# luciddreamer-cvlab/LucidDreamer

Hardware: AMD Instinct MI355X
Metric: views/sec fwd+bwd @1080p (1e6 Gaussians) (higher is better)
Workload: dtype f32

## Files before the change

### luciddreamer_amd/build.py

```python
import os
import shutil
import subprocess
import sys

_HERE = os.path.dirname(os.path.abspath(__file__))
CSRC = os.path.join(_HERE, "csrc")
LIBDIR = os.path.join(_HERE, "lib")
OBJDIR = os.path.join(LIBDIR, "obj")
LIB_PATH = os.path.join(LIBDIR, "liblucid_raster.so")
INCLUDE = os.path.join(os.path.dirname(_HERE), "include")

COMMON_FLAGS = ["--offload-arch=gfx950", "-O3", "-std=c++17", "-fPIC", "-munsafe-fp-atomics",
                "-fno-gpu-rdc", "-Wall", "-Wno-unused-function", "-I", INCLUDE]
SOURCES = {
    "preprocess.hip": ["-ffp-contract=off", "-fno-slp-vectorize"],
    "binning.hip": [],
    "tilebin.hip": [],
    "render_fwd.hip": ["-fno-slp-vectorize"],
    "render_bwd.hip": ["-fno-slp-vectorize"],
    "gauss_bwd.hip": [],
    "knn.hip": [],
    "loss.hip": ["-fno-slp-vectorize"],
    "rows.hip": [],
    "adam.hip": [],
    "mcmc.hip": [],
    "filter3d.hip": ["-ffp-contract=off"],
    "video.hip": ["-ffp-contract=off"],
    "api.hip": [],
}


def hipcc():
    for cand in (os.environ.get("HIPCC"), shutil.which("hipcc"), "/opt/rocm/bin/hipcc"):
        if cand and os.path.exists(cand):
            return cand
    raise RuntimeError("hipcc not found (need ROCm >= 7.0 with gfx950 support)")


def _stale(target, deps):
    if not os.path.exists(target):
        return True
    t = os.path.getmtime(target)
    return any(os.path.getmtime(d) > t for d in deps)


def source_hash():
    import hashlib
    h = hashlib.sha1()
    names = sorted(f for f in os.listdir(CSRC) if f.endswith((".hip", ".h", ".cpp")))
    for path in [os.path.join(CSRC, f) for f in names] + [os.path.join(INCLUDE, "lucid_raster.h")]:
        h.update(os.path.basename(path).encode())
        with open(path, "rb") as f:
            h.update(f.read())
    return h.hexdigest()[:12]


def _write_hash_header():
    path = os.path.join(OBJDIR, "lr_src_hash.h")
    text = f'#define LR_SRC_HASH "{source_hash()}"\n'
    old = open(path).read() if os.path.exists(path) else None
    if old != text:
        with open(path, "w") as f:
            f.write(text)
    return path


DIAG_LIBDIR = os.path.join(_HERE, "lib_diag")


def build(force=False, verbose=False, diagnostics=False):
    libdir = DIAG_LIBDIR if diagnostics else LIBDIR
    objdir = os.path.join(libdir, "obj")
    lib_path = os.path.join(libdir, "liblucid_raster.so")
    os.makedirs(objdir, exist_ok=True)
    os.makedirs(OBJDIR, exist_ok=True)
    cc = hipcc()
    hash_header = _write_hash_header()
    headers = [os.path.join(CSRC, "common.h"), os.path.join(CSRC, "gauss_bwd_body.h"), os.path.join(CSRC, "loss_ssim_fwd_body.h"),
               os.path.join(CSRC, "loss_ssim_bwd_body.h"), os.path.join(INCLUDE, "lucid_raster.h"), os.path.abspath(__file__)]
    objs = []
    procs = []
    for src, extra in SOURCES.items():
        sp = os.path.join(CSRC, src)
        op = os.path.join(objdir, src.replace(".hip", ".o"))
        if diagnostics:
            extra = extra + ["-DLR_DIAGNOSTICS"]
        objs.append(op)
        deps = [sp] + headers + ([hash_header] if src == "api.hip" else [])
        if force or _stale(op, deps):
            cmd = [cc, "-c", sp, "-o", op] + COMMON_FLAGS + ["-I", OBJDIR] + extra + os.environ.get("LR_EXTRA_HIPCC_FLAGS", "").split()
            if verbose:
                print(" ".join(cmd), flush=True)
            procs.append((src, subprocess.Popen(cmd, stdout=subprocess.PIPE, stderr=subprocess.STDOUT, text=True)))
    failed = []
    for src, p in procs:
        out, _ = p.communicate()
        if p.returncode != 0:
            failed.append((src, out))
        elif verbose and out.strip():
            print(out)
    if failed:
        raise RuntimeError("hipcc failed:\n" + "\n".join(f"--- {s} ---\n{o}" for s, o in failed))
    if force or procs or _stale(lib_path, objs):
        cmd = [cc, "-shared", "-fPIC", "--offload-arch=gfx950", "-o", lib_path] + objs
        if verbose:
            print(" ".join(cmd), flush=True)
        subprocess.check_call(cmd)
    return lib_path


EXT_SRC = os.path.join(CSRC, "torch_ext.cpp")


def ext_path():
    import sysconfig
    return os.path.join(_HERE, "_C_ext" + sysconfig.get_config_var("EXT_SUFFIX"))


def build_ext(force=False, verbose=False):
    import sysconfig
    import torch
    from torch.utils import cpp_extension as ce
    out = ext_path()
    deps = [EXT_SRC, os.path.join(INCLUDE, "lucid_raster.h"), os.path.abspath(__file__)]
    if not force and not _stale(out, deps):
        return out
    rocm = os.environ.get("ROCM_PATH", "/opt/rocm")
    cmd = ["g++", "-O2", "-std=c++17", "-fPIC", "-shared", "-w", EXT_SRC, "-o", out,
           "-DTORCH_EXTENSION_NAME=_C_ext", "-DTORCH_API_INCLUDE_EXTENSION_H", "-DUSE_ROCM", "-D__HIP_PLATFORM_AMD__",
           f"-D_GLIBCXX_USE_CXX11_ABI={int(torch._C._GLIBCXX_USE_CXX11_ABI)}", "-I", INCLUDE, "-I", os.path.join(rocm, "include"),
           "-I", sysconfig.get_paths()["include"]]
# ... 19 lines not shown
```

### luciddreamer_amd/csrc/api.hip

```cpp
#include "common.h"
#include "../../include/lucid_raster.h"
#include "lr_src_hash.h"

#include <cstdio>
#include <cstdlib>
#include <cstddef>
#include <cstring>
#include <cmath>
#include <map>
#include <atomic>
#include <chrono>
#include <mutex>
#include <thread>
#include <string>
#include <vector>

namespace {

thread_local std::string g_last_error;

int fail(int code, const std::string& msg)
{
    g_last_error = msg;
    return code;
// ... 15 lines not shown
            if (e__ == hipSuccess) e__ = hipGetLastError();                                       \
            if (e__ != hipSuccess)                                                                \
                return fail(LR_ERR_HIP, std::string("[HIP ERROR] after ") + what + ": " + hipGetErrorString(e__)); \
        }                                                                                         \
    } while (0)

enum Stage { ST_PREPROCESS = 0, ST_COMPACT, ST_BIN_COUNT, ST_BIN_SCAN, ST_BIN_SCATTER, ST_TILE_SORT, ST_RENDER_FWD,
             ST_GRAD_ZERO, ST_RENDER_BWD, ST_OUT_ZERO, ST_GAUSS_BWD, ST_COUNT };
const char* const kStageNames[ST_COUNT] = { "preprocess", "compact", "bin_count", "bin_scan", "bin_scatter", "tile_sort",
                                            "render_fwd", "grad_zero", "render_bwd", "out_zero", "gauss_bwd" };
struct ProfRec { int stage; hipEvent_t e0, e1; };
bool g_prof_on = false;
std::mutex g_prof_mu;
std::vector<ProfRec> g_prof_recs;
std::vector<hipEvent_t> g_prof_pool;

hipEvent_t prof_event()
{
    {
        std::lock_guard<std::mutex> lock(g_prof_mu);
        if (!g_prof_pool.empty()) { hipEvent_t e = g_prof_pool.back(); g_prof_pool.pop_back(); return e; }
    }
    hipEvent_t e = nullptr;
    (void)hipEventCreate(&e);
    return e;
}
struct ProfScope {
    hipStream_t s; ProfRec r; bool on;
    ProfScope(int stage, hipStream_t s_) : s(s_), on(g_prof_on)
    {
        if (on) { r.stage = stage; r.e0 = prof_event(); r.e1 = prof_event(); (void)hipEventRecord(r.e0, s); }
    }
    ~ProfScope()
    {
        if (on) { (void)hipEventRecord(r.e1, s); std::lock_guard<std::mutex> lock(g_prof_mu); g_prof_recs.push_back(r); }
    }
};

struct BinProf : lr::TileBinTimes {
    ProfRec cur; bool open = false;
    void mark(int boundary, hipStream_t s) override
    {
        if (!g_prof_on) return;
        if (open) { (void)hipEventRecord(cur.e1, s); std::lock_guard<std::mutex> lock(g_prof_mu); g_prof_recs.push_back(cur); open = false; }
        if (boundary < 4) {
            cur.stage = ST_BIN_COUNT + boundary; cur.e0 = prof_event(); cur.e1 = prof_event();
            (void)hipEventRecord(cur.e0, s); open = true;
        }
    }
};

struct TuneTable { int v[lr::TUNE_COUNT]; TuneTable() { for (int& x : v) x = -1; } } g_tune_table;
int* const g_tune = g_tune_table.v;
const char* const kTuneNames[] = { "bwd_red", "blend_quad", "tile_map", "preprocess", "gauss_bwd", "tsort", "walk_own", "hit_mask", "views_in_flight", "strict", "part_scan", "bwd_seg", "fwd_pair" };
static_assert(sizeof(kTuneNames) / sizeof(kTuneNames[0]) == lr::TUNE_COUNT, "one name per TuneKey");

std::mutex g_hint_mu;
std::map<std::pair<int, uint32_t>, float> g_vis_frac;
std::map<std::pair<int, uint32_t>, uint32_t> g_inst_hint;
constexpr float kSparseViewFraction = 0.30f;

void view_hint_note(int device, uint32_t P, uint32_t num_compact, uint32_t num_instances)
{
    if (P == 0) return;
    std::lock_guard<std::mutex> lock(g_hint_mu);
    g_vis_frac[std::make_pair(device, P)] = (float)num_compact / (float)P;
    g_inst_hint[std::make_pair(device, P)] = num_instances;
}
long long view_hint_instances(int device, uint32_t P)
{
    std::lock_guard<std::mutex> lock(g_hint_mu);
    auto it = g_inst_hint.find(std::make_pair(device, P));
    return it != g_inst_hint.end() ? (long long)it->second : -1;
}
bool view_hint_sparse(int device, uint32_t P)
{
    std::lock_guard<std::mutex> lock(g_hint_mu);
    auto it = g_vis_frac.find(std::make_pair(device, P));
    return it != g_vis_frac.end() && it->second <= kSparseViewFraction;
}

thread_local bool g_early_request = false;
thread_local long long g_early_ticket = -1;

struct StreamScratch { uint32_t* words = nullptr; size_t n = 0; bool dirty = false; };
std::mutex g_scratch_mu;
std::map<std::pair<int, hipStream_t>, StreamScratch> g_scratch;
StreamScratch* stream_scratch(hipStream_t s, size_t n_words)
{
    int device = 0;
    if (hipGetDevice(&device) != hipSuccess) return nullptr;
    StreamScratch* sc;
    {
        std::lock_guard<std::mutex> lock(g_scratch_mu);
        sc = &g_scratch[std::make_pair(device, s)];
    }
    if (sc->n < n_words) {
        uint32_t* w = nullptr;
        const size_t cap = n_words + n_words / 2 + 64;
        if (hipMalloc(reinterpret_cast<void**>(&w), cap * 4) != hipSuccess) return nullptr;
        if (hipMemsetAsync(w, 0, cap * 4, s) != hipSuccess) return nullptr;
        sc->words = w; sc->n = cap; sc->dirty = false;
    } else if (sc->dirty) {
        if (hipMemsetAsync(sc->words, 0, sc->n * 4, s) != hipSuccess) return nullptr;
        sc->dirty = false;
    }
    return sc;
// ... 130 lines not shown
    if (v.raw && M < 1) return fail(LR_ERR_INVALID_ARG, "raw mode: M = 1 + number of features_rest coefficients must be >= 1");
    if (P < 0 || width <= 0 || height <= 0) return fail(LR_ERR_INVALID_ARG, "P, width, height must be positive");
    if (!a.geom_alloc || !a.binning_alloc || !a.img_alloc) return fail(LR_ERR_INVALID_ARG, "allocator callbacks are required");
    if (!v.background || !v.viewmatrix || !v.projmatrix || !v.campos || !a.out_color || (!a.out_depth && !depth_optional))
        return fail(LR_ERR_INVALID_ARG, "background/viewmatrix/projmatrix/cam_pos/out_color/out_depth are required");
    if (P > 0 && (!v.means3D || !v.opacities || !radii)) return fail(LR_ERR_INVALID_ARG, "means3D/opacities/radii are required");
    if (P > 0 && v.shs == nullptr && v.colors_precomp == nullptr)
        return fail(LR_ERR_INVALID_ARG, "For non-RGB, provide precomputed Gaussian colors!");
    if (P > 0 && v.cov3D_precomp == nullptr && (v.scales == nullptr || v.rotations == nullptr))
        return fail(LR_ERR_INVALID_ARG, "provide scales+rotations or cov3D_precomp");
    if (v.shs != nullptr && (D < 0 || D > 3 || (D + 1) * (D + 1) > M))
        return fail(LR_ERR_INVALID_ARG, "SH degree must be 0..3 and (D+1)^2 <= M");
    if (binning_capacity < 0 || binning_capacity > 0xFFFFFFF0ll) return fail(LR_ERR_INVALID_ARG, "bad binning_capacity");

    const int gx = (width + TILE_X - 1) / TILE_X, gy = (height + TILE_Y - 1) / TILE_Y;
    const int num_tiles = gx * gy;

    const GeomLayout GL = geom_layout(P);
    const ImgLayout IL = img_layout(width, height);
    char* geom = a.geom_alloc(GL.total, a.geom_user);
    char* img = a.img_alloc(IL.total, a.img_user);
    if (!geom || !img) return fail(LR_ERR_ALLOC, "geom/img allocator returned NULL");

    GeomHeader* hdr = reinterpret_cast<GeomHeader*>(geom + GL.header);
    GaussRec* rec = reinterpret_cast<GaussRec*>(geom + GL.rec);
    uint8_t* clamped = reinterpret_cast<uint8_t*>(geom + GL.clamped);
    uint32_t* tiles_touched = reinterpret_cast<uint32_t*>(geom + GL.tiles_touched);
    uint32_t* vis_list = reinterpret_cast<uint32_t*>(geom + GL.vis_list);
    uint32_t* offsets = reinterpret_cast<uint32_t*>(geom + GL.offsets);
    uint4* hitrec = reinterpret_cast<uint4*>(geom + GL.hitrec);
    float* final_T = reinterpret_cast<float*>(img + IL.final_T);
    uint32_t* n_contrib = reinterpret_cast<uint32_t*>(img + IL.n_contrib);
    uint2* ranges = reinterpret_cast<uint2*>(img + IL.ranges);
    uint32_t* part_hist = reinterpret_cast<uint32_t*>(img + IL.part_hist);
    uint32_t* bin_total = reinterpret_cast<uint32_t*>(img + IL.bin_total);
    uint32_t* bin_start = reinterpret_cast<uint32_t*>(img + IL.bin_start);
    uint32_t* big_queue = reinterpret_cast<uint32_t*>(img + IL.big_queue);

    const size_t n_sum_words = chunk_sum_words(P);
    StreamScratch* scratch = P > 0 ? stream_scratch(s, n_sum_words) : nullptr;
    if (P > 0 && !scratch) return fail(LR_ERR_ALLOC, "could not allocate the per-stream scratch");
    struct DirtyOnError { StreamScratch* sc; bool armed; ~DirtyOnError() { if (sc && armed) sc->dirty = true; } } guard{ scratch, false };
    g_last_forward_ticket = -1;

    ViewParams vp;
    vp.view = v.viewmatrix; vp.proj = v.projmatrix; vp.campos = v.campos;
    vp.tan_fovx = v.tan_fovx; vp.tan_fovy = v.tan_fovy;
    vp.focal_y = height / (2.0f * v.tan_fovy);
    vp.focal_x = width / (2.0f * v.tan_fovx);
    vp.scale_modifier = v.scale_modifier;
    vp.W = width; vp.H = height; vp.gx = gx; vp.gy = gy; vp.P = P; vp.D = D; vp.M = M;
    vp.hit_origin_limit = tune_get(TUNE_HIT_MASK) == 0 ? 0 : HIT_ORIGIN_LIMIT;
    vp.raw = v.raw != 0; vp.sh_rest = v.sh_rest; vp.opacity_raw = nullptr; vp.dL_dsh_rest = nullptr;

    long long R_bound = 0;
    int num_rendered = 0;
    uint32_t* point_list = nullptr;
    uint32_t* inst_gid = nullptr;
    uint32_t* list_gid = nullptr;
    uint8_t* quad_hits = nullptr;
    uint2* seg_list = nullptr;
    float4* ckpt = nullptr;
    bool ranges_written = false;
    long long inst_hint = -1;

    if (P > 0) {
        int device = 0;
        (void)hipGetDevice(&device);
        inst_hint = view_hint_instances(device, (uint32_t)P);
        { ProfScope ps(ST_PREPROCESS, s);
        launch_preprocess(vp, v.means3D, v.scales, v.rotations, v.opacities, v.shs, v.cov3D_precomp, v.colors_precomp,
                          a.prefiltered != 0, radii, rec, clamped, tiles_touched, hitrec, nullptr, hdr,
                          (uint32_t)binning_capacity, scratch->words,
                          view_hint_sparse(device, (uint32_t)P), s, antialiasing); }
        guard.armed = true;
        LR_DEBUG_SYNC(debug, s, "preprocess");

        uint32_t* log_slot = nullptr;
        uint32_t log_tag = 0;
#ifdef LR_DIAGNOSTICS
        static const bool no_log = [] { const char* e = getenv("LR_NO_FWD_LOG"); return e && atoi(e) != 0; }();
#else
        constexpr bool no_log = false;
#endif
        if (binning_capacity != 0 && !no_log) {
            if (ForwardLog* L = forward_log(device)) {
                const long long seq = L->next.fetch_add(1);
                log_slot = L->dev + (size_t)(seq % kLogSlots) * kLogWords;
                log_tag = (uint32_t)(seq + 1);
                g_last_forward_ticket = ((long long)device << 41) | kLogTicketBit | (seq & (kLogTicketBit - 1));
            }
        }
        { ProfScope ps(ST_COMPACT, s);
        launch_compact(P, tiles_touched, reinterpret_cast<const uint4*>(scratch->words), vis_list, offsets, hdr,
                       (uint32_t)binning_capacity, log_slot, log_tag, bin_total, (uint32_t)part_plan(num_tiles).bins, reset_sticky, s); }
        LR_DEBUG_SYNC(debug, s, "compact");

        if (binning_capacity == 0) {
            uint32_t meta[9];
            LR_HIP_CHECK(hipMemcpyAsync(meta, hdr, sizeof(meta), hipMemcpyDeviceToHost, s));
            LR_HIP_CHECK(hipStreamSynchronize(s));
            view_hint_note(device, (uint32_t)P, meta[8], meta[6]);
            R_bound = meta[6];
            if (meta[0] > 0x7FFFFFFFu)
                return fail(LR_ERR_INVALID_ARG, "num_rendered exceeds INT_MAX: use async mode (binning_capacity > 0) and read the count with lr_check");
            num_rendered = (int)meta[0];
// ... 58 lines not shown
    using namespace lr;
    const bool antialiasing = g_antialiasing.load(std::memory_order_relaxed) != 0;
    const lr_view& v = a.view;
    const int P = v.P, M = v.M, width = v.width, height = v.height, debug = a.debug;
    const bool raw = v.raw != 0;
    char* const geom_buffer = a.geom_buffer; char* const binning_buffer = a.binning_buffer; char* const image_buffer = a.image_buffer;
    const unsigned int accumulate_mask = a.accumulate_mask;
    const bool depth = a.dL_depths != nullptr && a.depth_image != nullptr;
    hipStream_t s = reinterpret_cast<hipStream_t>(a.stream);
    if (P <= 0) return 0;
    if (!geom_buffer || !binning_buffer || !image_buffer) return fail(LR_ERR_INVALID_ARG, "scratch buffers are required");
    if (!a.dL_dpix || !a.dL_dmean2D || !a.dL_dopacity || !a.dL_dmean3D)
        return fail(LR_ERR_INVALID_ARG, "gradient outputs dL_dmean2D/dL_dopacity/dL_dmean3D are required");
    if (v.colors_precomp != nullptr && !a.dL_dcolor) return fail(LR_ERR_INVALID_ARG, "dL_dcolor is required with colors_precomp");
    if (v.cov3D_precomp != nullptr && !a.dL_dcov3D) return fail(LR_ERR_INVALID_ARG, "dL_dcov3D is required with cov3D_precomp");
    if (v.scales != nullptr && (!a.dL_dscale || !a.dL_drot)) return fail(LR_ERR_INVALID_ARG, "dL_dscale/dL_drot are required with scales");
    if (v.shs != nullptr && a.dL_dsh == nullptr) return fail(LR_ERR_INVALID_ARG, "dL_dsh is required when shs is given");
    {
        const void* g16[11] = { a.dL_dmean2D, a.dL_dconic, a.dL_dopacity, a.dL_dcolor, a.dL_dmean3D, a.dL_dcov3D, a.dL_dsh, a.dL_dscale,
                                a.dL_drot, a.dL_dsh_rest, a.dL_dmean2D_abs };
        for (const void* p : g16)
            if ((reinterpret_cast<uintptr_t>(p) & 15u) != 0)
                return fail(LR_ERR_INVALID_ARG, "gradient outputs must be 16-byte aligned");
    }

    const int gx = (width + TILE_X - 1) / TILE_X, gy = (height + TILE_Y - 1) / TILE_Y;
    const GeomLayout GL = geom_layout(P);
    const ImgLayout IL = img_layout(width, height);
    const GaussRec* rec = reinterpret_cast<const GaussRec*>(geom_buffer + GL.rec);
    const uint8_t* clamped = reinterpret_cast<const uint8_t*>(geom_buffer + GL.clamped);
    const uint32_t* offsets = reinterpret_cast<const uint32_t*>(geom_buffer + GL.offsets);
    const uint32_t* vis_list = reinterpret_cast<const uint32_t*>(geom_buffer + GL.vis_list);
    const GeomHeader* hdr = reinterpret_cast<const GeomHeader*>(geom_buffer + GL.header);
    const float* final_T = reinterpret_cast<const float*>(image_buffer + IL.final_T);
    const uint32_t* n_contrib = reinterpret_cast<const uint32_t*>(image_buffer + IL.n_contrib);
    const uint2* ranges = reinterpret_cast<const uint2*>(image_buffer + IL.ranges);

    const uint32_t* point_list = reinterpret_cast<const uint32_t*>(binning_buffer);
    const long long seg_bound = (a.binning_capacity > 0 || a.R > 0)
                                    ? bin_seg_capacity(a.binning_capacity > 0 ? a.binning_capacity : (long long)a.R) : -1;

    ViewParams vp;
    vp.view = v.viewmatrix; vp.proj = v.projmatrix; vp.campos = v.campos;
    vp.tan_fovx = v.tan_fovx; vp.tan_fovy = v.tan_fovy;
    vp.focal_y = height / (2.0f * v.tan_fovy);
    vp.focal_x = width / (2.0f * v.tan_fovx);
    vp.scale_modifier = v.scale_modifier;
    vp.W = width; vp.H = height; vp.gx = gx; vp.gy = gy; vp.P = P; vp.D = v.D; vp.M = M;
    vp.hit_origin_limit = tune_get(TUNE_HIT_MASK) == 0 ? 0 : HIT_ORIGIN_LIMIT;
    vp.raw = raw;
    vp.sh_rest = raw ? v.sh_rest : nullptr;
    vp.opacity_raw = raw ? v.opacities : nullptr;
    vp.dL_dsh_rest = raw ? a.dL_dsh_rest : nullptr;

    { ProfScope ps(ST_RENDER_BWD, s);
    launch_render_bwd(width, height, gx, gy, ranges, point_list, rec, v.background, final_T, n_contrib, a.dL_dpix,
                      binning_buffer, hdr, reinterpret_cast<const uint32_t*>(image_buffer + IL.tile_seg0),
                      reinterpret_cast<const float4*>(image_buffer + IL.c_final), seg_bound, s,
                      depth ? a.dL_depths : nullptr, depth ? a.depth_image : nullptr, a.dL_dalpha, a.dL_dmean2D_abs != nullptr || stat_abs); }
    LR_DEBUG_SYNC(debug, s, "render backward");
    if (debug) {
        uint32_t uncovered = 0;
        LR_HIP_CHECK(hipMemcpy(&uncovered, &hdr->bwd_uncovered, 4, hipMemcpyDeviceToHost));
        if (uncovered) return fail(LR_ERR_INVALID_ARG, kUncoveredMsg);
    }
    if (wait_before_accumulate != nullptr) LR_HIP_CHECK(hipStreamWaitEvent(s, wait_before_accumulate, 0));
    {
        const unsigned long long Pn = (unsigned long long)P;
        float* ptrs[9] = { a.dL_dmean2D, a.dL_dconic, a.dL_dopacity, a.dL_dcolor, a.dL_dmean3D, a.dL_dcov3D, a.dL_dsh, a.dL_dscale, a.dL_drot };
        const unsigned long long nsh = raw ? 3 * Pn : (unsigned long long)M * 3 * Pn;
        const unsigned long long nf[9] = { 3 * Pn, 4 * Pn, Pn, 3 * Pn, 3 * Pn, 6 * Pn, nsh, 3 * Pn, 4 * Pn };
        float* zp[11]; unsigned long long zn[11]; int zc = 0;
        const bool no_fill = (accumulate_mask & LR_ACC_NO_ZERO_FILL) != 0u;
        for (int k = 0; k < 9; k++)
            if (ptrs[k] != nullptr && !((accumulate_mask >> k) & 1u) && (!no_fill || k == ACC_MEAN2D)) { zp[zc] = ptrs[k]; zn[zc] = nf[k]; zc++; }
        if (!no_fill && raw && a.dL_dsh_rest != nullptr && M > 1 && !((accumulate_mask >> ACC_SH) & 1u) && zc < 9) {
            zp[zc] = a.dL_dsh_rest; zn[zc] = (unsigned long long)(M - 1) * 3 * Pn; zc++;
        }
        const bool abs_own = a.dL_dmean2D_abs != nullptr && zc >= 9;
        if (a.dL_dmean2D_abs != nullptr && !abs_own) { zp[zc] = a.dL_dmean2D_abs; zn[zc] = 3 * Pn; zc++; }
        if (zc > 0) {
            ProfScope ps(ST_OUT_ZERO, s);
            launch_zero_outputs(zp, zn, zc, s);
            if (abs_own) { float* one = a.dL_dmean2D_abs; const unsigned long long n = 3 * Pn; launch_zero_outputs(&one, &n, 1, s); }
        }
    }
    { ProfScope ps(ST_GAUSS_BWD, s);
    launch_gauss_bwd(vp, v.means3D, v.scales, v.rotations, v.shs, v.cov3D_precomp, v.colors_precomp, vis_list, clamped, offsets,
                     binning_buffer, hdr,
                     a.dL_dmean2D, a.dL_dconic, a.dL_dopacity, a.dL_dcolor, a.dL_dmean3D, a.dL_dcov3D, a.dL_dsh, a.dL_dscale,
                     a.dL_drot, accumulate_mask, acc16, s, depth, antialiasing, a.dL_dmean2D_abs, stat_accum, stat_abs); }
    LR_DEBUG_SYNC(debug, s, "preprocess backward");
    LR_HIP_CHECK(hipGetLastError());
    return 0;
}

static int check_backward(const lr_backward_args& a)
{
    const lr_view& v = a.view;
    if (const int rc = check_view(v)) return rc;
    if (!v.raw && a.dL_dsh_rest) return fail(LR_ERR_INVALID_ARG, "dL_dsh_rest goes with raw mode only");
    if (v.P > 0 && a.dL_depths != nullptr && a.depth_image == nullptr)
        return fail(LR_ERR_INVALID_ARG, "lr_view_backward: dL_depths needs the forward's depth image");
    if (v.raw && v.P > 0 && (!a.dL_dsh || (v.M > 1 && !a.dL_dsh_rest)))
        return fail(LR_ERR_INVALID_ARG, "raw mode needs dL_dfeatures_dc and dL_dfeatures_rest");
    return 0;
// ... 995 lines not shown
```

### luciddreamer_amd/csrc/common.h

```cpp
#pragma once
#include <hip/hip_runtime.h>
#include <stdint.h>
#include <stddef.h>

namespace lr {

constexpr int TILE_X = 16;
constexpr int TILE_Y = 16;
constexpr int TILE_PIX = TILE_X * TILE_Y;
constexpr int WAVE = 64;

struct __attribute__((aligned(16))) GaussRec {
    float x, y, ca, cb;
    float cc, opacity, r, g;
    float b, depth, qmax, pad1;
};
static_assert(sizeof(GaussRec) == 48, "GaussRec must be 48 bytes");

struct __attribute__((aligned(16))) GradRec {
    float dmx, dmy, dca, dcb;
    float dcc, dop, dr, dg;
    float db, pad0, pad1, pad2;
};
static_assert(sizeof(GradRec) == 48, "GradRec must be 48 bytes");

constexpr uint32_t HIT_MASK_TILES = 64;
constexpr int HIT_ORIGIN_LIMIT = 4096;
__host__ __device__ inline uint32_t hit_geo(int minx, int miny, int rw, uint32_t area, int origin_limit)
{
    return (area <= HIT_MASK_TILES && minx < origin_limit && miny < origin_limit)
               ? ((uint32_t)minx | ((uint32_t)miny << 12) | ((uint32_t)rw << 24)) : 0u;
}

struct GeomHeader {
    uint32_t num_rendered;
    uint32_t overflow;
    uint32_t prefilter_trap;
    uint32_t capacity;
    uint32_t P;
    uint32_t num_sorted;
    uint32_t num_instances;
    uint32_t bin_bound;
    uint32_t num_compact;
    uint32_t n_seg;
    uint32_t bwd_uncovered;
    uint32_t reserved[49];
    uint32_t sticky_overflow;
    uint32_t reserved_tail[3];
};
static_assert(sizeof(GeomHeader) == 256, "GeomHeader must be 256 bytes");

__device__ __forceinline__ void lds_barrier()
{
    asm volatile("s_waitcnt lgkmcnt(0)" ::: "memory");
    __syncthreads();
}
// ... 153 lines not shown
    return t * dy;
}
__device__ __forceinline__ float gauss_power1(float Ap, float Bd, float Cdd, float dx)
{
    return __builtin_fmaf(__builtin_fmaf(Ap, dx, Bd), dx, Cdd);
}
template <bool STRICT>
__device__ __forceinline__ void gauss_row(float qB, float qC, float dy, float& r0, float& r1)
{
    if (STRICT) { r0 = dy; r1 = 0.f; }
    else { r0 = gauss_bd(qB, dy); r1 = gauss_cdd(qC, dy); }
}
__device__ __forceinline__ float gauss_power_strict(float ca, float cb, float cc, float dx, float dy)
{
#pragma clang fp contract(off)
    return -0.5f * (ca * dx * dx + cc * dy * dy) - cb * dx * dy;
}
__device__ __forceinline__ float strict_expf(float x)
{
#pragma clang fp contract(off)
    const float c = 0x1.715476p+0f, cc = 0x1.4ae0bep-26f;
    const float ph = x * c;
    const float pl = __builtin_fmaf(x, cc, __builtin_fmaf(x, c, -ph));
    const float e = __builtin_rintf(ph);
    const float a = (ph - e) + pl;
    return __builtin_ldexpf(__builtin_amdgcn_exp2f(a), (int)e);
}
template <bool STRICT>
__device__ __forceinline__ float gauss_weight(float qA, float qB, float qC, float r0, float r1, float dx, float& power)
{
    if (STRICT) {
        power = gauss_power_strict(qA, qB, qC, dx, r0);
        return strict_expf(power);
    }
    power = gauss_power1(qA, r0, r1, dx);
    return __builtin_amdgcn_exp2f(power);
}

constexpr float LOG2E = 1.4426950408889634f;
constexpr float LN2 = 0.6931471805599453f;
__device__ __forceinline__ float gauss_exp2(float power2) { return __builtin_amdgcn_exp2f(power2); }

struct ViewParams {
    const float* view;
    const float* proj;
    const float* campos;
    float tan_fovx, tan_fovy, focal_x, focal_y, scale_modifier;
    int W, H, gx, gy, P, D, M;
    int hit_origin_limit;
    int raw;
    const float* sh_rest;
    const float* opacity_raw;
    float* dL_dsh_rest;
};

__device__ __forceinline__ float act_scale(float s) { return expf(s); }
__device__ __forceinline__ float act_opacity(float o) { return 1.0f / (1.0f + expf(-o)); }
__device__ __forceinline__ float act_quat_inv_norm(float r, float x, float y, float z)
{
    return 1.0f / fmaxf(sqrtf(r * r + x * x + y * y + z * z), 1e-12f);
}

void launch_preprocess(const ViewParams& vp, const float* means3D, const float* scales, const float* rotations,
                       const float* opacities, const float* shs, const float* cov3D_precomp,
                       const float* colors_precomp, bool prefiltered, int* radii, GaussRec* rec,
                       uint8_t* clamped, uint32_t* tiles_touched, uint4* hitrec, uint32_t* depth_key,
                       GeomHeader* hdr, uint32_t binning_capacity, uint32_t* chunk_sums, bool sparse_view_hint, hipStream_t s,
                       bool antialiasing = false);
inline size_t chunk_sum_words(int P) { return 4 * (((size_t)(P > 0 ? P : 1) + SCAN_TILE - 1) / SCAN_TILE) + 1; }
void launch_mark_visible(int P, const float* means3D, const float* view, const float* proj, uint8_t* present,
                         hipStream_t s);

inline int radix_sort_passes(int end_bit) { return (end_bit + RADIX_BITS - 1) / RADIX_BITS; }
void radix_sort_pairs(uint32_t* key_a, uint32_t* key_b, uint32_t* val_a, uint32_t* val_b, bool vals_iota,
                      const uint32_t* n_dev, long long n_bound, int end_bit, uint32_t* hist,
                      uint32_t** keys_out, uint32_t** vals_out, hipStream_t s);

void launch_compact(int P, const uint32_t* tiles_touched, const uint4* block_sums,
                    uint32_t* vis_list, uint32_t* offsets, GeomHeader* hdr, uint32_t capacity, uint32_t* log_slot,
                    uint32_t log_tag, uint32_t* zero_words, uint32_t n_zero, bool reset_sticky, hipStream_t s);
struct TileBinTimes { virtual void mark(int boundary, hipStream_t s) = 0; virtual ~TileBinTimes() {} };
int launch_tile_binning(int P, int gx, int gy, int slot_bits, const uint32_t* vis_list, const uint32_t* offsets,
                        const uint4* hitrec, const GaussRec* rec, const int* radii, GeomHeader* hdr,
                        uint32_t* part_hist, uint32_t* bin_total, uint32_t* bin_start, uint32_t* big_queue,
                        uint32_t* inst_gid, unsigned long long* words, uint32_t* point_list, uint32_t* list_gid, uint2* ranges,
                        long long bin_bound_hint, TileBinTimes* t, uint32_t* clear_words, uint32_t n_clear, hipStream_t s);

enum TuneKey { TUNE_BWD_RED = 0, TUNE_BLEND_QUAD, TUNE_TILE_MAP, TUNE_PREPROCESS, TUNE_GAUSS_BWD, TUNE_TSORT, TUNE_WALK_OWN, TUNE_HIT_MASK, TUNE_VIEWS_IN_FLIGHT, TUNE_STRICT, TUNE_PART_SCAN, TUNE_BWD_SEG, TUNE_FWD_PAIR, TUNE_COUNT };
int tune_get(int key);

enum { BLEND_HALF = 0, BLEND_QUAD = 1, BLEND_TILE = 2 };
int blend_shape(int num_tiles, long long inst_bound = -1);
struct ViewsInFlight { explicit ViewsInFlight(int n); ~ViewsInFlight(); int prev; };
int views_in_flight();
void note_fwd_shape(int shape);
int last_fwd_shape();
int last_bwd_shape();
enum { TILE_MAP_BANDS = 0, TILE_MAP_PLAIN = 1 };
int blend_tile_map(int num_tiles);
__device__ __forceinline__ int blend_tile(int map, int num_tiles)
{
    int t = (int)blockIdx.x;
    if (map == TILE_MAP_BANDS) {
        const int per = (num_tiles + 7) >> 3;
        t = (int)(blockIdx.x & 7) * per + (int)(blockIdx.x >> 3);
    }
    return t < num_tiles ? t : -1;
}
void launch_render_fwd(int W, int H, int gx, int gy, const uint2* ranges, const uint32_t* point_list,
                       const uint32_t* list_gid, const GaussRec* rec, const float* bg, float* final_T,
                       uint32_t* n_contrib, float* out_color, float* out_depth, uint8_t* quad_hits,
                       GeomHeader* hdr, uint2* seg_list, float4* ckpt, uint32_t* tile_seg0, float4* c_final,
                       long long inst_hint, hipStream_t s);
void launch_render_alpha(const float* final_T, long long n, float* alpha, hipStream_t s);
void launch_render_bwd(int W, int H, int gx, int gy, const uint2* ranges, const uint32_t* point_list,
                       const GaussRec* rec, const float* bg, const float* final_T,
                       const uint32_t* n_contrib, const float* dL_dpix, char* bin_base, const GeomHeader* hdr,
                       const uint32_t* tile_seg0, const float4* c_final, long long seg_bound, hipStream_t s,
                       const float* dL_ddepth = nullptr, const float* depth_img = nullptr, const float* dL_dalpha = nullptr,
                       bool absgrad = false);
__device__ __forceinline__ void adam_one(float gi, float& mi, float& vi, float& pi, float w1, float beta2, float w2,
                                         float bc2_sqrt, float eps, float step_size)
{
    mi = __builtin_fmaf(w1, gi - mi, mi);
    vi = vi * beta2;
    vi = __builtin_fmaf(w2 * gi, gi, vi);
    const float denom = sqrtf(vi) / bc2_sqrt + eps;
    pi = __builtin_fmaf(-step_size, mi / denom, pi);
}
void launch_gauss_bwd(const ViewParams& vp, const float* means3D, const float* scales, const float* rotations,
                      const float* shs, const float* cov3D_precomp, const float* colors_precomp,
                      const uint32_t* vis_list, const uint8_t* clamped, const uint32_t* offsets,
                      const char* bin_base, const GeomHeader* hdr,
                      float* dL_dmean2D, float* dL_dconic, float* dL_dopacity, float* dL_dcolor,
                      float* dL_dmean3D, float* dL_dcov3D, float* dL_dsh, float* dL_dscale, float* dL_drot,
                      uint32_t accum_mask, float* acc16, hipStream_t s, bool depth = false, bool antialiasing = false,
                      float* dL_dmean2D_abs = nullptr, float* stat_accum = nullptr, bool stat_abs = false);
void launch_uninterleave_add(int P, const float* acc16, float* mean2D, float* opacity, float* mean3D, float* scale, float* rot,
                             hipStream_t s, float* stat_accum = nullptr);
size_t select_workspace_bytes(int P);
int launch_select_rows(int P, const uint8_t* mask, int n_tensors, const void* const* src, void* const* dst,
// ... 82 lines not shown
```

### luciddreamer_amd/csrc/preprocess.hip

```cpp
#include <cstddef>
#include "common.h"

namespace lr {

namespace {

__device__ constexpr float SH_C0 = 0.28209479177387814f;
__device__ constexpr float SH_C1 = 0.4886025119029199f;
__device__ constexpr float SH_C2[5] = { 1.0925484305920792f, -1.0925484305920792f, 0.31539156525252005f,
                                        -1.0925484305920792f, 0.5462742152960396f };
__device__ constexpr float SH_C3[7] = { -0.5900435899266435f, 2.890611442640554f, -0.4570457994644658f,
                                        0.3731763325901154f, -0.4570457994644658f, 1.445305721320277f,
                                        -0.5900435899266435f };

struct M3 { float c[3][3]; };

__device__ __forceinline__ M3 m3_mul(const M3& A, const M3& B)
{
    M3 R;
#pragma unroll
    for (int j = 0; j < 3; j++)
#pragma unroll
        for (int i = 0; i < 3; i++)
            R.c[j][i] = A.c[0][i] * B.c[j][0] + A.c[1][i] * B.c[j][1] + A.c[2][i] * B.c[j][2];
// ... 373 lines not shown
        rgb.x = colors_precomp[3 * (size_t)idx]; rgb.y = colors_precomp[3 * (size_t)idx + 1];
        rgb.z = colors_precomp[3 * (size_t)idx + 2];
    } else {
        const size_t li = (size_t)idx;
        V3 dir = { means3D[3 * li] - vp.campos[0], means3D[3 * li + 1] - vp.campos[1], means3D[3 * li + 2] - vp.campos[2] };
        const float len = sqrtf(dir.x * dir.x + dir.y * dir.y + dir.z * dir.z);
        dir.x = dir.x / len; dir.y = dir.y / len; dir.z = dir.z / len;
        switch (vp.D) {
            case 0: rgb = eval_sh<0>(shs, RAW ? vp.sh_rest : nullptr, idx, vp.M, dir, cbits); break;
            case 1: rgb = eval_sh<1>(shs, RAW ? vp.sh_rest : nullptr, idx, vp.M, dir, cbits); break;
            case 2: rgb = eval_sh<2>(shs, RAW ? vp.sh_rest : nullptr, idx, vp.M, dir, cbits); break;
            default: rgb = eval_sh<3>(shs, RAW ? vp.sh_rest : nullptr, idx, vp.M, dir, cbits); break;
        }
    }
    clamped[idx] = cbits;

    float opacity = RAW ? act_opacity(opacities[idx]) : opacities[idx];
    if constexpr (AA) opacity = opacity * pj.coef;
    qmax = cull_qmax(opacity);
    float4* dst = reinterpret_cast<float4*>(rec + idx);
    dst[0] = make_float4(pj.pix, pj.piy, pj.con_a, pj.con_b);
    dst[1] = make_float4(pj.con_c, opacity, rgb.x, rgb.y);
    dst[2] = make_float4(rgb.z, pj.vz, qmax, 0.f);
}

template <bool RAW, bool AA>
__global__ void __launch_bounds__(PL_THREADS) __attribute__((amdgpu_waves_per_eu(RAW ? 4 : 5, 8)))
k_preprocess_pool(ViewParams vp, const float* __restrict__ means3D, const float* __restrict__ scales,
                  const float* __restrict__ rotations, const float* __restrict__ opacities,
                  const float* __restrict__ shs, const float* __restrict__ cov3D_precomp,
                  const float* __restrict__ colors_precomp, int prefiltered,
                  int* __restrict__ radii, GaussRec* __restrict__ rec, uint8_t* __restrict__ clamped,
                  uint32_t* __restrict__ tiles_touched, uint4* __restrict__ hitrec, GeomHeader* hdr,
                  uint32_t binning_capacity, uint32_t* __restrict__ chunk_sums)
{
    __shared__ uint16_t s_near[PL_POOL];
    __shared__ int s_radius[PL_POOL];
    __shared__ uint32_t s_tiles[PL_POOL];
    __shared__ float s_mid[6][PL_POOL];
    __shared__ float s_coef[AA ? PL_POOL : 1];
    __shared__ uint32_t s_mid_id[PL_POOL];
    __shared__ uint32_t s_tests[PL_POOL];
    __shared__ uint2 s_rect[PL_POOL];
    __shared__ uint32_t s_mask[PL_POOL][2];
    __shared__ uint32_t s_wcnt[PL_ROUNDS * PL_WAVES];
    __shared__ uint32_t s_nmid;
    __shared__ uint32_t s_sum[3];
    const int tid = threadIdx.x, w = tid >> 6, l = tid & 63;
    const int base = blockIdx.x * PL_POOL;
    uint32_t* const trap = chunk_sums != nullptr ? chunk_sums + 4 * ((size_t)(vp.P + SCAN_TILE - 1) / SCAN_TILE) : &hdr->prefilter_trap;
    if (tid == 0) { s_nmid = 0u; s_sum[0] = 0u; s_sum[1] = 0u; s_sum[2] = 0u; }
    const float* __restrict__ V = vp.view;

    bool pass[PL_ROUNDS];
    uint64_t m[PL_ROUNDS];
#pragma unroll
    for (int r = 0; r < PL_ROUNDS; r++) {
        const int loc = r * PL_THREADS + tid, gid = base + loc;
        const bool in_range = gid < vp.P;
        const size_t li = in_range ? (size_t)gid : 0;
        const float vz1 = V[2] * means3D[3 * li] + V[6] * means3D[3 * li + 1] + V[10] * means3D[3 * li + 2] + V[14];
        pass[r] = in_range && !(vz1 <= 0.2f);
        if (in_range && !pass[r] && prefiltered) *trap = 1;
        s_radius[loc] = 0; s_tiles[loc] = 0u;
        m[r] = __ballot(pass[r]);
        if (l == 0) s_wcnt[r * PL_WAVES + w] = (uint32_t)__popcll(m[r]);
    }
    lds_barrier();
    uint32_t n_near = 0;
#pragma unroll
    for (int r = 0; r < PL_ROUNDS; r++) {
        uint32_t before = n_near;
#pragma unroll
        for (int i = 0; i < PL_WAVES; i++) { if (i < w) before += s_wcnt[r * PL_WAVES + i]; n_near += s_wcnt[r * PL_WAVES + i]; }
        if (pass[r]) s_near[before + __popcll(m[r] & ((1ull << l) - 1ull))] = (uint16_t)(r * PL_THREADS + tid);
    }
    lds_barrier();

    for (uint32_t i0 = 0; i0 < n_near; i0 += PL_THREADS) {
        const uint32_t i = i0 + (uint32_t)tid;
        Projected pj;
        bool ok = false;
        uint32_t loc = 0;
        if (i < n_near) {
            loc = s_near[i];
            ok = project_gaussian<RAW, AA>(vp, base + (int)loc, means3D, scales, rotations, cov3D_precomp, pj);
        }
        const uint64_t mk = __ballot(ok);
        uint32_t wbase = 0;
        if (l == 0 && mk != 0ull) wbase = atomicAdd(&s_nmid, (uint32_t)__popcll(mk));
        wbase = (uint32_t)__shfl((int)wbase, 0);
        if (ok) {
            const uint32_t slot = wbase + (uint32_t)__popcll(mk & ((1ull << l) - 1ull));
            s_mid[0][slot] = pj.pix; s_mid[1][slot] = pj.piy; s_mid[2][slot] = pj.con_a; s_mid[3][slot] = pj.con_b;
            s_mid[4][slot] = pj.con_c; s_mid[5][slot] = pj.vz;
            if constexpr (AA) s_coef[slot] = pj.coef;
            s_mid_id[slot] = loc; s_radius[loc] = pj.radius;
        }
    }
    lds_barrier();

    const uint32_t n_mid = s_nmid;
    uint32_t my_ref = 0;
    for (uint32_t i0 = 0; i0 < n_mid; i0 += PL_THREADS) {
        const uint32_t i = i0 + (uint32_t)tid;
        uint32_t tests = 0;
        if (i < n_mid) {
            Projected pj;
            pj.pix = s_mid[0][i]; pj.piy = s_mid[1][i]; pj.con_a = s_mid[2][i]; pj.con_b = s_mid[3][i];
            pj.con_c = s_mid[4][i]; pj.vz = s_mid[5][i];
            if constexpr (AA) pj.coef = s_coef[i];
            const uint32_t loc = s_mid_id[i];
            pj.radius = s_radius[loc];
            int minx, miny, width; uint32_t area; float qmax;
            colour_and_record<RAW, AA>(vp, base + (int)loc, pj, means3D, opacities, shs, colors_precomp, rec, clamped,
                                   minx, miny, width, area, qmax);
// ... 135 lines not shown
```

Before: 6075.

## Add conservative screen-space cull before preprocess compaction

Adds a cheap conservative test in the preprocess prepass that projects each Gaussian's centre and bounds its footprint using the max scale and quaternion norm. Gaussians that provably cannot touch any tile are dropped before the expensive per-Gaussian projection and covariance work. The scale and rotation loads are hoisted into a prefetch loop for all rounds. This adds memory traffic for scales and rotations plus register pressure, and the bound must stay conservative to keep results correct. The cull is on by default, can be disabled through a new tune key, and is disabled on the backward view.

```diff
diff --git a/luciddreamer_amd/build.py b/luciddreamer_amd/build.py
--- a/luciddreamer_amd/build.py
+++ b/luciddreamer_amd/build.py
@@ -76,7 +76,7 @@
     os.makedirs(OBJDIR, exist_ok=True)
     cc = hipcc()
     hash_header = _write_hash_header()
-    headers = [os.path.join(CSRC, "common.h"), os.path.join(CSRC, "gauss_bwd_body.h"), os.path.join(CSRC, "loss_ssim_fwd_body.h"),
+    headers = [os.path.join(CSRC, "common.h"), os.path.join(CSRC, "screen_cull.h"), os.path.join(CSRC, "gauss_bwd_body.h"), os.path.join(CSRC, "loss_ssim_fwd_body.h"),
                os.path.join(CSRC, "loss_ssim_bwd_body.h"), os.path.join(INCLUDE, "lucid_raster.h"), os.path.abspath(__file__)]
     objs = []
     procs = []
diff --git a/luciddreamer_amd/csrc/api.hip b/luciddreamer_amd/csrc/api.hip
--- a/luciddreamer_amd/csrc/api.hip
+++ b/luciddreamer_amd/csrc/api.hip
@@ -91,7 +91,7 @@
 
 struct TuneTable { int v[lr::TUNE_COUNT]; TuneTable() { for (int& x : v) x = -1; } } g_tune_table;
 int* const g_tune = g_tune_table.v;
-const char* const kTuneNames[] = { "bwd_red", "blend_quad", "tile_map", "preprocess", "gauss_bwd", "tsort", "walk_own", "hit_mask", "views_in_flight", "strict", "part_scan", "bwd_seg", "fwd_pair" };
+const char* const kTuneNames[] = { "bwd_red", "blend_quad", "tile_map", "preprocess", "gauss_bwd", "tsort", "walk_own", "hit_mask", "views_in_flight", "strict", "part_scan", "bwd_seg", "fwd_pair", "pcull" };
 static_assert(sizeof(kTuneNames) / sizeof(kTuneNames[0]) == lr::TUNE_COUNT, "one name per TuneKey");
 
 std::mutex g_hint_mu;
@@ -328,6 +328,8 @@
     vp.W = width; vp.H = height; vp.gx = gx; vp.gy = gy; vp.P = P; vp.D = D; vp.M = M;
     vp.hit_origin_limit = tune_get(TUNE_HIT_MASK) == 0 ? 0 : HIT_ORIGIN_LIMIT;
     vp.raw = v.raw != 0; vp.sh_rest = v.sh_rest; vp.opacity_raw = nullptr; vp.dL_dsh_rest = nullptr;
+    vp.cull = screen_cull_view(width, height, gx, gy, vp.tan_fovx, vp.tan_fovy, vp.focal_x, vp.focal_y);
+    vp.pcull = tune_get(TUNE_PCULL) == 0 ? 0 : 1;
 
     long long R_bound = 0;
     int num_rendered = 0;
@@ -492,6 +494,7 @@
     vp.sh_rest = raw ? v.sh_rest : nullptr;
     vp.opacity_raw = raw ? v.opacities : nullptr;
     vp.dL_dsh_rest = raw ? a.dL_dsh_rest : nullptr;
+    vp.cull = ScreenCull{}; vp.pcull = 0;
 
     { ProfScope ps(ST_RENDER_BWD, s);
     launch_render_bwd(width, height, gx, gy, ranges, point_list, rec, v.background, final_T, n_contrib, a.dL_dpix,
diff --git a/luciddreamer_amd/csrc/common.h b/luciddreamer_amd/csrc/common.h
--- a/luciddreamer_amd/csrc/common.h
+++ b/luciddreamer_amd/csrc/common.h
@@ -2,6 +2,7 @@
 #include <hip/hip_runtime.h>
 #include <stdint.h>
 #include <stddef.h>
+#include "screen_cull.h"
 
 namespace lr {
 
@@ -261,6 +262,8 @@
     const float* sh_rest;
     const float* opacity_raw;
     float* dL_dsh_rest;
+    ScreenCull cull;
+    int pcull;
 };
 
 __device__ __forceinline__ float act_scale(float s) { return expf(s); }
@@ -295,7 +298,7 @@
                         uint32_t* inst_gid, unsigned long long* words, uint32_t* point_list, uint32_t* list_gid, uint2* ranges,
                         long long bin_bound_hint, TileBinTimes* t, uint32_t* clear_words, uint32_t n_clear, hipStream_t s);
 
-enum TuneKey { TUNE_BWD_RED = 0, TUNE_BLEND_QUAD, TUNE_TILE_MAP, TUNE_PREPROCESS, TUNE_GAUSS_BWD, TUNE_TSORT, TUNE_WALK_OWN, TUNE_HIT_MASK, TUNE_VIEWS_IN_FLIGHT, TUNE_STRICT, TUNE_PART_SCAN, TUNE_BWD_SEG, TUNE_FWD_PAIR, TUNE_COUNT };
+enum TuneKey { TUNE_BWD_RED = 0, TUNE_BLEND_QUAD, TUNE_TILE_MAP, TUNE_PREPROCESS, TUNE_GAUSS_BWD, TUNE_TSORT, TUNE_WALK_OWN, TUNE_HIT_MASK, TUNE_VIEWS_IN_FLIGHT, TUNE_STRICT, TUNE_PART_SCAN, TUNE_BWD_SEG, TUNE_FWD_PAIR, TUNE_PCULL, TUNE_COUNT };
 int tune_get(int key);
 
 enum { BLEND_HALF = 0, BLEND_QUAD = 1, BLEND_TILE = 2 };
diff --git a/luciddreamer_amd/csrc/preprocess.hip b/luciddreamer_amd/csrc/preprocess.hip
--- a/luciddreamer_amd/csrc/preprocess.hip
+++ b/luciddreamer_amd/csrc/preprocess.hip
@@ -449,16 +449,45 @@
     if (tid == 0) { s_nmid = 0u; s_sum[0] = 0u; s_sum[1] = 0u; s_sum[2] = 0u; }
     const float* __restrict__ V = vp.view;
 
+    const bool cull_on = vp.pcull != 0 && cov3D_precomp == nullptr;
+    const float* __restrict__ Pm = vp.proj;
+    const float kv9 = cull_on ? screen_cull_kv9(vp.cull, V) : 0.0f;
     bool pass[PL_ROUNDS];
     uint64_t m[PL_ROUNDS];
+    float mean[PL_ROUNDS][3], scl[PL_ROUNDS][3];
+    float4 rot[PL_ROUNDS];
+#pragma unroll
+    for (int r = 0; r < PL_ROUNDS; r++) {
+        const int gid = base + r * PL_THREADS + tid;
+        const size_t li = gid < vp.P ? (size_t)gid : 0;
+#pragma unroll
+        for (int k = 0; k < 3; k++) mean[r][k] = means3D[3 * li + k];
+        if (cull_on) {
+#pragma unroll
+            for (int k = 0; k < 3; k++) scl[r][k] = scales[3 * li + k];
+            rot[r] = reinterpret_cast<const float4*>(rotations)[li];
+        }
+    }
 #pragma unroll
     for (int r = 0; r < PL_ROUNDS; r++) {
         const int loc = r * PL_THREADS + tid, gid = base + loc;
         const bool in_range = gid < vp.P;
-        const size_t li = in_range ? (size_t)gid : 0;
-        const float vz1 = V[2] * means3D[3 * li] + V[6] * means3D[3 * li + 1] + V[10] * means3D[3 * li + 2] + V[14];
-        pass[r] = in_range && !(vz1 <= 0.2f);
-        if (in_range && !pass[r] && prefiltered) *trap = 1;
+        const float px_w = mean[r][0], py_w = mean[r][1], pz_w = mean[r][2];
+        const float vz1 = V[2] * px_w + V[6] * py_w + V[10] * pz_w + V[14];
+        const bool near = in_range && !(vz1 <= 0.2f);
+        if (in_range && !near && prefiltered) *trap = 1;
+        bool culled = false;
+        if (cull_on) {
+            float sx = scl[r][0], sy = scl[r][1], sz = scl[r][2];
+            float qr = rot[r].x, qx = rot[r].y, qy = rot[r].z, qz = rot[r].w;
+            if (RAW) {
+                sx = act_scale(sx); sy = act_scale(sy); sz = act_scale(sz);
+                const float inv = act_quat_inv_norm(qr, qx, qy, qz);
+                qr *= inv; qx *= inv; qy *= inv; qz *= inv;
+            }
+            culled = screen_cull_point(vp.cull, kv9, Pm, vp.scale_modifier, px_w, py_w, pz_w, vz1, sx, sy, sz, qr, qx, qy, qz);
+        }
+        pass[r] = near && !culled;
         s_radius[loc] = 0; s_tiles[loc] = 0u;
         m[r] = __ballot(pass[r]);
         if (l == 0) s_wcnt[r * PL_WAVES + w] = (uint32_t)__popcll(m[r]);
diff --git a/luciddreamer_amd/csrc/screen_cull.h b/luciddreamer_amd/csrc/screen_cull.h
--- /dev/null
+++ b/luciddreamer_amd/csrc/screen_cull.h
@@ -0,0 +1,74 @@
+#pragma once
+
+#if defined(__HIPCC__) || defined(__CUDACC__)
+#define LR_SC_HD __host__ __device__ __forceinline__
+#else
+#define LR_SC_HD inline
+#endif
+
+namespace lr {
+
+constexpr float SC_PIX_MARGIN = 2.0f;
+constexpr float SC_NINE = 9.0f * 1.001f;
+constexpr float SC_C0 = 0.9163f;
+constexpr float SC_S_MAX = 1e9f;
+
+struct ScreenCull {
+    float g;
+    float half_w, half_h;
+    float kx, ex;
+    float ky, ey;
+};
+
+inline ScreenCull screen_cull_view(int W, int H, int gx, int gy, float tan_fovx, float tan_fovy, float focal_x, float focal_y)
+{
+    const float limx = 1.3f * tan_fovx, limy = 1.3f * tan_fovy;
+    ScreenCull c;
+    c.g = focal_x * focal_x * (1.0f + limx * limx) + focal_y * focal_y * (1.0f + limy * limy);
+    c.half_w = 0.5f * (float)W; c.half_h = 0.5f * (float)H;
+    const float m_lo = SC_PIX_MARGIN - 0.5f;
+    const float m_hx = 16.0f * (float)gx + 1.5f + SC_PIX_MARGIN, m_hy = 16.0f * (float)gy + 1.5f + SC_PIX_MARGIN;
+    c.kx = 0.5f * (m_hx - m_lo); c.ex = 0.5f * (m_hx + m_lo);
+    c.ky = 0.5f * (m_hy - m_lo); c.ey = 0.5f * (m_hy + m_lo);
+    return c;
+}
+
+LR_SC_HD float screen_cull_wf(const float* V)
+{
+    return V[0] * V[0] + V[1] * V[1] + V[2] * V[2] + V[4] * V[4] + V[5] * V[5] + V[6] * V[6] + V[8] * V[8] + V[9] * V[9] +
+           V[10] * V[10];
+}
+
+LR_SC_HD float screen_cull_scale(float scale_modifier, float sx, float sy, float sz)
+{
+    const float mx = __builtin_fmaxf(__builtin_fmaxf(__builtin_fabsf(sx), __builtin_fabsf(sy)), __builtin_fabsf(sz));
+    return __builtin_fabsf(scale_modifier) * mx + (sx + sy + sz) * 0.0f;
+}
+
+LR_SC_HD float screen_cull_qn2(float r, float x, float y, float z) { return r * r + x * x + y * y + z * z; }
+
+LR_SC_HD bool screen_cull_reject(const ScreenCull& c, float kv9, float hx, float hy, float hwp, float vz, float s, float qn2)
+{
+    const float rb = qn2 + __builtin_fabsf(1.0f - qn2);
+    const float sr = s * rb;
+    const float a9 = (hwp * hwp) * ((SC_NINE * SC_C0) * (vz * vz) + kv9 * (sr * sr));
+    const float ux = __builtin_fabsf((hx + hwp) * c.half_w - c.kx * hwp) - c.ex * hwp;
+    const float uy = __builtin_fabsf((hy + hwp) * c.half_h - c.ky * hwp) - c.ey * hwp;
+    const float bx = vz * ux, by = vz * uy;
+    const bool off = ((bx > 0.0f) & (a9 < bx * bx)) | ((by > 0.0f) & (a9 < by * by));
+    return off & (hwp > 0.0f) & (vz > 0.0f) & (sr <= SC_S_MAX);
+}
+
+LR_SC_HD bool screen_cull_point(const ScreenCull& c, float kv9, const float* Pm, float scale_modifier, float px_w, float py_w,
+                                float pz_w, float vz, float sx, float sy, float sz, float qr, float qx, float qy, float qz)
+{
+    const float hx = Pm[0] * px_w + Pm[4] * py_w + Pm[8] * pz_w + Pm[12];
+    const float hy = Pm[1] * px_w + Pm[5] * py_w + Pm[9] * pz_w + Pm[13];
+    const float hw = Pm[3] * px_w + Pm[7] * py_w + Pm[11] * pz_w + Pm[15];
+    return screen_cull_reject(c, kv9, hx, hy, hw + 0.0000001f, vz, screen_cull_scale(scale_modifier, sx, sy, sz),
+                              screen_cull_qn2(qr, qx, qy, qz));
+}
+
+LR_SC_HD float screen_cull_kv9(const ScreenCull& c, const float* V) { return SC_NINE * c.g * screen_cull_wf(V); }
+
+}
```

Result: faster. 6137 (median of 6 runs) (+1.0%).
